# Yalt8826/WeatherForecast_STGCN_MAML

Measured on AMD Instinct MI355X. Metric: MAML meta-steps/sec (15-task batch, N=441, T=24), higher is better.
Workload: dtype f32

## Files before the change

weatherforecast_stgcn_maml_amd/_capi.py:

```python
from __future__ import annotations

import ctypes
import os
import threading

import numpy as np

HERE = os.path.dirname(os.path.abspath(__file__))
LIB_PATH = os.environ.get("SMAML_LIB") or os.path.join(HERE, "libsmaml.so")

EXPORTS = (
    "smaml_last_error", "smaml_abi_version", "smaml_build_info", "smaml_param_layout", "smaml_graph_ell",
    "smaml_create", "smaml_destroy", "smaml_set_graph", "smaml_set_gcn_params", "smaml_reserve",
    "smaml_workspace_bytes", "smaml_so_kept_steps", "smaml_set_dropout", "smaml_set_task_ids", "smaml_gcn_conv", "smaml_forward", "smaml_set_tasks",
    "smaml_meta_step", "smaml_adamw_step", "smaml_adapt_steps", "smaml_timing", "smaml_timing_collect",
    "smaml_backward", "smaml_gcn_forward", "smaml_lstm_forward", "smaml_lstm_backward", "smaml_head_loss",
    "smaml_clip_sgd", "smaml_inner_loop", "smaml_alloc", "smaml_free", "smaml_comm_unique_id",
    "smaml_comm_init", "smaml_comm_allreduce", "smaml_comm_destroy", "smaml_variant_counts", "smaml_set_option",
    "smaml_dropout", "smaml_sync", "smaml_gcn_conv_ex", "smaml_gcn_conv_backward", "smaml_relu_mask",
    "smaml_adapt_prepare", "smaml_adapt_phases",
)
ABI_VERSION = 7
GCN_RELU, GCN_PLAIN = 1, 2

VARIANTS = ("fwd", "fwd_drop", "fwd_split", "fwd_img", "fwd_dual", "fwd_dual_kept", "fwd_dual_img", "bwd_big", "bwd_small", "bwd_split",
            "bwd_dual_big", "bwd_dual_big_kept", "bwd_dual_small", "bwd_dual_small_kept", "wgrad", "wgrad_wide", "wgrad_pair",
            "fwd_kw", "bwd_kw", "gcn_dedup", "xg_dedup", "wgrad_dedup", "f_compact")

TIMING_CATEGORIES = ("gcn_layer", "lstm_fwd_step", "lstm_fwd_dual", "head_loss", "head_dh", "lstm_bwd_step",
                     "lstm_bwd_dual", "wgrad", "wgrad_reduce", "misc", "xg_proj", "dg_rowsum",
                     "lstm_fwd_step_wall", "lstm_fwd_dual_wall", "lstm_bwd_step_wall", "lstm_bwd_dual_wall")

ERRORS = {1: "EINVAL", 2: "EHIP", 3: "ENOMEM", 4: "ESTATE", 5: "ENOTIMPL"}


class SmamlError(RuntimeError):
    def __init__(self, code, msg):
        super().__init__(f"smaml error {ERRORS.get(code, code)}: {msg}")
        self.code = code


class Dims(ctypes.Structure):
    _fields_ = [(n, ctypes.c_int32) for n in (
        "num_nodes", "window_size", "input_channels", "hidden_channels", "lstm_hidden_size",
        "lstm_num_layers", "forecast_horizon", "output_channels")]

    @classmethod
    def from_model(cls, d):
        return cls(d.num_nodes, d.window_size, d.input_channels, d.hidden_channels,
                   d.lstm_hidden_size, d.lstm_num_layers, d.forecast_horizon, d.output_channels)
# ... 64 lines not shown
def lib():
    global _lib
    with _lock:
        if _lib is None:
            if not os.path.exists(LIB_PATH):
                raise SmamlError(-1, f"{LIB_PATH} not built; run __graft_entry__.build()")
            L = ctypes.CDLL(LIB_PATH)
            L.smaml_abi_version.restype = I32
            if L.smaml_abi_version() != ABI_VERSION:
                raise SmamlError(-1, f"{LIB_PATH} has ABI {L.smaml_abi_version()}, expected {ABI_VERSION}; rebuild")
            for name, (args, res) in _SIGS.items():
                fn = getattr(L, name)
                fn.argtypes = args
                fn.restype = res
            _lib = L
    return _lib


def build_info() -> str:
    return lib().smaml_build_info().decode()


def product_forms() -> dict:
    tail = build_info().split(":", 1)[1]
    return {k: int(v) for k, v in (kv.split("=") for kv in tail.split())}


def check(rc):
    if rc != 0:
        raise SmamlError(rc, lib().smaml_last_error().decode(errors="replace"))


def param_layout(dims, which: int):
    L = lib()
    d = Dims.from_model(dims)
    cap = 64
    offs = (ctypes.c_int64 * cap)()
    sizes = (ctypes.c_int64 * cap)()
    cnt = ctypes.c_int32()
    tot = ctypes.c_int64()
    check(L.smaml_param_layout(ctypes.byref(d), which, offs, sizes, cap, ctypes.byref(cnt),
                               ctypes.byref(tot)))
    return [(offs[i], sizes[i]) for i in range(cnt.value)], tot.value


def graph_ell(edge_index: np.ndarray, num_nodes: int):
    L = lib()
# ... 217 lines not shown
```

weatherforecast_stgcn_maml_amd/csrc/api.cpp:

```cpp
#include <hip/hip_runtime.h>

#include <algorithm>
#include <array>
#include <chrono>
#include <cmath>
#include <dlfcn.h>
#include <cstdlib>
#include <cstring>
#include <string>
#include <thread>
#include <vector>

#include "kernels.h"
#include "smaml.h"

using namespace smaml;

namespace {

thread_local std::string g_err;

int fail(int code, const std::string& msg) {
  g_err = msg;
  return code;
// ... 161 lines not shown
};

}

static Knobs default_knobs() {
  Knobs k;
  k.bwd_big_min = SMAML_BWD_BIG_MIN;
  k.bwdd_big_min = SMAML_BWDD_BIG_MIN;
  k.split_max = SMAML_SPLIT_MAX;
  k.wgrad_group_max_rows = SMAML_WGRAD_GROUP_ROWS;
  k.wgrad_group_wgs = SMAML_WGRAD_GROUP_WGS;
  k.gcn_fused = SMAML_GCN_FUSED;
  k.gate_img = SMAML_GATE_IMG;
  k.wgrad_wide = 1;
  k.wgrad_pair = SMAML_WGRAD_PAIR;
  k.bwdd_remap = SMAML_BWDD_REMAP_DEFAULT;
  k.small_kw = SMAML_SMALL_KW;
  k.gcn_dedup = 1;
  k.xg_dedup = SMAML_XG_DEDUP_DEFAULT;
  k.wgrad_dedup = SMAML_WGRAD_DEDUP_DEFAULT;
  k.bptt_streams = SMAML_BPTT_STREAMS_DEFAULT;
  k.fwd_streams = SMAML_FWD_STREAMS_DEFAULT;
  k.f_compact = SMAML_F_COMPACT_DEFAULT;
  return k;
}

enum { AD_RESERVE = 0, AD_ALLOC, AD_FILL, AD_STEPS, AD_NPH };
struct AdPhases {
  double ms[AD_NPH] = {};
  int64_t filled = 0;
};

struct smaml_ctx {
  smaml_dims dims{};
  Dims d{};
  ParamOff po{};
  GcnOff go{};
  int device = 0;
  int32_t* ell_c = nullptr;
  float* ell_v = nullptr;
  int32_t *tr_p = nullptr, *tr_c = nullptr;
  float* tr_v = nullptr;
  int64_t tr_nnz_cap = 0;
  float* bw_scratch = nullptr;
  int64_t bw_scratch_cap = 0;
  const float* gcn = nullptr;
// ... 1689 lines not shown
    c->kn.wgrad_group_max_rows = (int)std::min<int64_t>(value, 1 << 30);
  } else if (k == "gcn_fused" && (value == 0 || value == 1)) {
    c->kn.gcn_fused = (int)value;
  } else if (k == "gate_img" && (value == 0 || value == 1)) {
    c->kn.gate_img = (int)value;
  } else if (k == "wgrad_wide" && (value == 0 || value == 1)) {
    c->kn.wgrad_wide = (int)value;
  } else if (k == "wgrad_pair" && (value == 0 || value == 1)) {
    c->kn.wgrad_pair = (int)value;
  } else if (k == "bwdd_remap" && (value == 0 || value == 1)) {
    c->kn.bwdd_remap = (int)value;
  } else if (k == "small_kw" && value >= 0 && value <= 2) {
    c->kn.small_kw = (int)value;
  } else if (k == "gcn_dedup" && (value == 0 || value == 1)) {
    c->kn.gcn_dedup = (int)value;
  } else if (k == "xg_dedup" && (value == 0 || value == 1)) {
    c->kn.xg_dedup = (int)value;
  } else if (k == "wgrad_dedup" && (value == 0 || value == 1)) {
    c->kn.wgrad_dedup = (int)value;
  } else if (k == "bptt_streams" && value >= 1 && value <= 4) {
    c->kn.bptt_streams = (int)value;
  } else if (k == "f_compact" && (value == 0 || value == 1)) {
    c->kn.f_compact = (int)value;
  } else if (k == "fwd_streams" && value >= 0 && value <= 4) {
    c->kn.fwd_streams = (int)value;
  } else if (k == "adapt_phase_sync" && (value == 0 || value == 1)) {
    c->ad_phase_sync = (int)value;
  } else if (k == "adapt_gcn_batch" && value >= 0 && value <= 256) {
    c->ad_gcn_batch = (int)value;
  } else if (k == "wgrad_group_wgs" && value >= 1) {
    c->kn.wgrad_group_wgs = (int)std::min<int64_t>(value, 1 << 20);
  } else if (k == "grid_barrier" && (value == 0 || value == 1)) {
    c->bar_fused = (int)value;
  } else if (k == "barrier_timeout_us" && value >= 1) {
    c->bar_timeout_us = std::min<int64_t>(value, 600000000);
  } else if (k == "comm_timeout_ms" && value >= 1) {
    c->comm_timeout_ms = std::min<int64_t>(value, 3600000);
  } else if (k == "barrier_oversize" && value >= 0 && value <= 64) {
    c->bar_oversize = (int)value;
  } else if (k == "keep" && value >= -1) {
    c->keep_max = (int)std::min<int64_t>(value, 1 << 20);
    c->keep_tried_K = -1;
  } else {
    return fail(SMAML_EINVAL, "unknown option or bad value: " + k);
  }
  return SMAML_OK;
// ... 333 lines not shown
```

weatherforecast_stgcn_maml_amd/csrc/kernels.h:

```cpp
#pragma once
#include <hip/hip_runtime.h>
#include <stdint.h>

namespace smaml {

constexpr int ELLW = 8;
constexpr int MAX_LAYERS = 8;

struct Dims {
  int N = 0;
  int T = 0;
  int Cin0 = 0;
  int Hc = 0;
  int H = 0;
  int L = 0;
  int Hf = 0;
  int C = 0;
  int HfC = 0;
};

struct LayerOff {
  int64_t wih = 0, whh = 0, bih = 0, bhh = 0;
  int cin = 0;
};
// ... 39 lines not shown
  V_FWD = 0,
  V_FWD_DROP,
  V_FWD_SPLIT,
  V_FWD_IMG,
  V_FWDD,
  V_FWDD_KEPT,
  V_FWDD_IMG,
  V_BWD_BIG,
  V_BWD_SMALL,
  V_BWD_SPLIT,
  V_BWDD_BIG,
  V_BWDD_BIG_KEPT,
  V_BWDD_SMALL,
  V_BWDD_SMALL_KEPT,
  V_WGRAD,
  V_WGRAD_WIDE,
  V_WGRAD_PAIR,
  V_FWD_KW,
  V_BWD_KW,
  V_GCN_DEDUP,
  V_XG_DEDUP,
  V_WGRAD_DEDUP,
  V_F_COMPACT,
  NVAR
};

#ifndef SMAML_BWD_BIG_MIN
#define SMAML_BWD_BIG_MIN (3 * 256)
#endif
#ifndef SMAML_BWDD_BIG_MIN
#define SMAML_BWDD_BIG_MIN (3 * 256)
#endif
#ifndef SMAML_SPLIT_MAX
#define SMAML_SPLIT_MAX 4
#endif

struct Knobs {
  int bwd_big_min = 0;
  int bwdd_big_min = 0;
  int split_max = 1;
  int wgrad_group_max_rows = 0;
  int wgrad_group_wgs = 1;
  int gcn_fused = 0;
  int gate_img = 0;
  int wgrad_wide = 0;
  int wgrad_pair = 0;
  int bwdd_remap = 0;
  int small_kw = 0;
  int gcn_dedup = 0;
  int xg_dedup = 0;
  int wgrad_dedup = 0;
  int bptt_streams = 1;
  int fwd_streams = 0;
  int f_compact = 0;
};
#ifndef SMAML_GATE_IMG
#define SMAML_GATE_IMG 1
#endif
#ifndef SMAML_GCN_FUSED
#define SMAML_GCN_FUSED 1
#endif
#ifndef SMAML_BWDD_REMAP_DEFAULT
#define SMAML_BWDD_REMAP_DEFAULT 1
#endif
#ifndef SMAML_SMALL_KW
#define SMAML_SMALL_KW 1
#endif
#ifndef SMAML_XG_DEDUP_DEFAULT
#define SMAML_XG_DEDUP_DEFAULT 1
#endif
#ifndef SMAML_WGRAD_DEDUP_DEFAULT
#define SMAML_WGRAD_DEDUP_DEFAULT 1
#endif
#ifndef SMAML_BPTT_STREAMS_DEFAULT
#define SMAML_BPTT_STREAMS_DEFAULT 2
#endif
#ifndef SMAML_F_COMPACT_DEFAULT
#define SMAML_F_COMPACT_DEFAULT 1
#endif
#ifndef SMAML_FWD_STREAMS_DEFAULT
#define SMAML_FWD_STREAMS_DEFAULT 0
#endif
#ifndef SMAML_WGRAD_PAIR
#define SMAML_WGRAD_PAIR 1
#endif
#ifndef SMAML_WGRAD_GROUP_ROWS
#define SMAML_WGRAD_GROUP_ROWS 2048
#endif
#ifndef SMAML_WGRAD_GROUP_WGS
#define SMAML_WGRAD_GROUP_WGS 256
#endif

constexpr int GATE_IMG_BYTES = 3 * 128 * 16 * 2;
struct GateImgs {
  char* th = nullptr;
  char* u = nullptr;
  int64_t tstride = 0;
  int64_t off[MAX_LAYERS][2] = {};
};
constexpr int BWD_IMG_BYTES = 3 * 32 * 16 * 2;
struct BwdImgs {
// ... 97 lines not shown
inline int grid_barrier_grid(int cap, int items, int oversize) {
  if (cap <= 0 || items <= 0) return 0;
  if (oversize > 0) return cap * oversize + 1;
  const int q = cap / 4 > 0 ? cap / 4 : 1;
  return items < q ? items : q;
}
int grid_barrier_blocks(const void* fn, int items, int oversize);
int grid_barrier_capacity(const void* fn);
#ifndef SMAML_WGRAD_MAXSPLIT
#define SMAML_WGRAD_MAXSPLIT 128
#endif

struct FwdWave {
  int n = 0;
  int l[MAX_LAYERS] = {}, t[MAX_LAYERS] = {}, off[MAX_LAYERS + 1] = {};
  LayerOff lo[MAX_LAYERS] = {};
  int tm0 = 0, ntm = 0;
};
struct BwdWave {
  int n = 0;
  int l[MAX_LAYERS] = {}, t[MAX_LAYERS] = {}, off[MAX_LAYERS + 1] = {};
  LayerOff lo[MAX_LAYERS] = {};
  int64_t wih_up[MAX_LAYERS] = {};
  int tm0 = 0;
};
double bwd_wave(const Dims& d, const Work& w, const ParamOff& po, int e, int blocks_per_problem, bool dual,
                BwdWave& wv);
double fwd_wave(const Dims& d, const Work& w, const ParamOff& po, int diag, int blocks_per_problem, bool dual,
                FwdWave& wv);

const char* products_info();

void launch_gcn_layer(hipStream_t s, const Dims& d, int layer, int Zb, int B, const float* const* xtab,
                      const float* src, float* dst, bool remap_lstm, bool relu, const float* W,
                      const float* b, int cin, int cout, const int* ell_c, const float* ell_v, int rows_per_sample,
                      int ell_rows, const Drop* drop = nullptr, int drop_rps = 0);

struct FastDiv {
  uint64_t m = 0;
  uint32_t s = 0;
  uint32_t d = 0;
  FastDiv() = default;
  __host__ explicit FastDiv(uint32_t dd) : d(dd) {
    s = 0;
    while ((1ull << s) < dd) ++s;
    m = (uint64_t)((((unsigned __int128)1 << (32 + s)) + dd - 1) / dd);
  }
  __device__ __forceinline__ uint32_t div(uint32_t n) const {
    return (uint32_t)(((unsigned __int128)n * m) >> (32 + s));
  }
// ... 147 lines not shown
```

weatherforecast_stgcn_maml_amd/csrc/kernels.hip:

```cpp
#include <cmath>
#include <mutex>
#include <utility>
#include <vector>

#include "kernels.h"
#include "loaders.h"

namespace smaml {

using CfgNT = GemmCfg<128, 128, 2, 2, true, true, 32, SMAML_X6_BWD>;
using CfgGate = GemmCfg<32 * SMAML_GATE_WM, 128 * SMAML_GATE_WN, SMAML_GATE_WM, SMAML_GATE_WN, true, true, SMAML_GATE_BK, SMAML_X6_GATE,
                        SMAML_GATE_NST>;
using CfgGateP = GemmCfg<128, 128 * SMAML_GATE_WN, 4, SMAML_GATE_WN, true, true, SMAML_GATE_BK, SMAML_X6_GATE>;
using CfgNN = GemmCfg<64, 128, 2, 2, true, false, SMAML_NN_BK, SMAML_X6_BWD>;
using CfgTN = GemmCfg<SMAML_TN_BM, SMAML_TN_BN, SMAML_TN_WM, SMAML_TN_WN, false, false, SMAML_TN_BK, SMAML_X6_WGRAD,
                      SMAML_TN_NST, false>;

__device__ __forceinline__ float block_sum(float v, float* red) {
#pragma unroll
  for (int o = 32; o > 0; o >>= 1) v += __shfl_xor(v, o, 64);
  const int lane = threadIdx.x & 63, wave = threadIdx.x >> 6;
  __syncthreads();
  if (lane == 0) red[wave] = v;
  __syncthreads();
// ... 1076 lines not shown
void launch_head_dh(hipStream_t s, const Dims& d, const Work& w, const float* theta, int64_t tstride,
                    const ParamOff& po) {
  dim3 grid((w.M + CfgNN::BM - 1) / CfgNN::BM, (d.H + CfgNN::BN - 1) / CfgNN::BN, w.Z);
  k_gemm_nn<<<grid, CfgNN::NTH, 0, s>>>(w.dpred, (int64_t)w.M * d.HfC, w.M, d.HfC, theta, tstride, po.wo, d.H,
                                w.dH, (int64_t)w.M * d.H);
  if (w.drop.lstm()) launch_drop_rows(s, w, d.H, w.dH, (int64_t)w.M * d.H, w.dH);
}

using CfgNNs = GemmCfg<64, 64, 2, 2, true, false, SMAML_NN_BK, SMAML_X6_BWD>;
using CfgBwd = GemmCfg<SMAML_BWD_BM, 128, SMAML_BWD_WM, SMAML_BWD_WN, true, false, SMAML_NN_BK, SMAML_X6_BWD,
                       SMAML_BWD_NST>;

double bwd_wave(const Dims& d, const Work& w, const ParamOff& po, int e, int blocks_per_problem, bool dual,
                BwdWave& wv) {
  double fl = 0.0;
  int n = 0, off = 0;
  for (int l = d.L - 1; l >= 0; --l) {
    const int t = d.T - 1 - (e - (d.L - 1 - l));
    if (t < 0 || t >= d.T) continue;
    wv.l[n] = l;
    wv.t[n] = t;
    wv.lo[n] = po.lay[l];
    wv.wih_up[n] = l + 1 < d.L ? po.lay[l + 1].wih : 0;
    wv.off[n] = off;
    off += blocks_per_problem;
    ++n;
    const int segs = (l + 1 < d.L ? 1 : 0) + (t + 1 < d.T ? 1 : 0);
    fl += (dual ? 3.0 : 1.0) * 2.0 * w.Z * w.M * 4 * d.H * d.H * segs;
  }
  wv.n = n;
  for (int q = n; q <= MAX_LAYERS; ++q) wv.off[q] = off;
  return fl;
}

#ifndef SMAML_DIAG_BWD
#define SMAML_DIAG_BWD 0
#endif
#ifndef SMAML_EPI_DEPTH
#define SMAML_EPI_DEPTH 1
#endif
template <class C>
constexpr int epi_smem_floats() {
  constexpr int E = SMAML_BWD_HALFEPI ? C::BM * C::BN / 2 : C::BM * C::BN;
  return C::SMEM_FLOATS > E ? C::SMEM_FLOATS : E;
}

// ... 93 lines not shown
    for (int h = 0; h < 2; ++h) {
      if (h) __syncthreads();
      acc_to_lds_half<CfgNN>(acc, smem, h);
      const int mh = m0 + h * HC::BM;
      if (mh + HC::BM <= M && n0 + HC::BN <= H)
        bwd_cell_<H, HC, HEAD, false>(smem, Gz, dGz, dhz, Cz, dHz, dcz, mh, n0, t, T, M);
      else
        bwd_cell_<H, HC, HEAD, true>(smem, Gz, dGz, dhz, Cz, dHz, dcz, mh, n0, t, T, M);
    }
  } else {
    acc_to_lds<CfgNN>(acc, smem);
    if (m0 + CfgNN::BM <= M && n0 + CfgNN::BN <= H)
      bwd_cell_<H, CfgNN, HEAD, false>(smem, Gz, dGz, dhz, Cz, dHz, dcz, m0, n0, t, T, M);
    else
      bwd_cell_<H, CfgNN, HEAD, true>(smem, Gz, dGz, dhz, Cz, dHz, dcz, m0, n0, t, T, M);
  }
}

template <int H, class CfgNN, bool DROP>
__global__ SMAML_BWD_ATTR __launch_bounds__(CfgNN::NTH) void k_lstm_bwd_step(const float* GsAll, float* dGAll,
                                                      float* __restrict__ dhAll, const float* __restrict__ CsAll,
                                                      const float* __restrict__ dHhead, float* __restrict__ dcAll,
                                                      int64_t lsz, const float* __restrict__ theta, int64_t tstride,
                                                      BwdWave wv, int L, int T, int M, Drop dr) {
  __shared__ float smem[epi_smem_floats<CfgNN>()];
  constexpr int G4 = 4 * H;
  const Blk bk = xcd_block();
  int mb;
  const int p = bwd_block(wv, bk.x, mb);
  mb += wv.tm0;
  const int l = wave_sel(wv.l, p), t = wave_sel(wv.t, p);
  const LayerOff lo = wave_sel(wv.lo, p);
  const int64_t wih_up = wave_sel(wv.wih_up, p);
  const int z = bk.z;
  const int m0 = mb * CfgNN::BM, n0 = bk.y * CfgNN::BN;
  const int64_t slab = (int64_t)z * T * M;
  const float* th = theta + (int64_t)z * tstride;
  const float* Gz = GsAll + (int64_t)l * lsz * 4 + slab * G4;
  float* dGz = dGAll + (int64_t)l * lsz * 4 + slab * G4;
  float* dhz = dhAll ? dhAll + (int64_t)l * lsz + slab * H : nullptr;
  const float* Cz = CsAll + (int64_t)l * lsz + slab * H;
  float* dcz = dcAll + ((int64_t)l * gridDim.z + z) * M * H;
  Acc<CfgNN> acc;
  acc.zero();
  {
    const bool up = l + 1 < L, nx = t + 1 < T;
    const float* pa = dGAll + (int64_t)(l + 1) * lsz * 4 + (slab + (int64_t)t * M) * G4;
    const float* pn = dGz + (int64_t)(t + 1) * M * G4;
    const int ns = (up ? 1 : 0) + (nx ? 1 : 0);
    if (DROP && up) {
      const XDrop xd{drop_site(dr.seed, 2, dr.step, l), dr.thr_lstm, dr.sc_lstm,
                     ((uint64_t)dr.task_id[z] * T + t) * M * H, H};
      gemm_mainloop<CfgNN>(SegKC{{pa, nullptr, nullptr, nullptr}, {G4, 0, 0, 0}, M},
                           SegMC{{th + wih_up, nullptr}, {G4, 0}, H}, m0, n0, 0, G4, acc, smem);
      drop_acc<CfgNN>(acc, xd, m0, n0);
      if (nx)
        gemm_mainloop<CfgNN>(SegKC{{pn, nullptr, nullptr, nullptr}, {G4, 0, 0, 0}, M},
                             SegMC{{th + lo.whh, nullptr}, {G4, 0}, H}, m0, n0, 0, G4, acc, smem);
    } else {
      const SegKCt<2> la{{up ? pa : pn, pn}, {G4, G4}, M};
      const SegMCt<2> lb{{up ? th + wih_up : th + lo.whh, th + lo.whh}, {G4, G4}, H};
      if (ns && SMAML_DIAG_BWD != 2) gemm_mainloop<CfgNN>(la, lb, m0, n0, 0, ns * G4, acc, smem);
    }
  }
  if (SMAML_DIAG_BWD == 1) {
    acc_to_lds<CfgNN>(acc, smem);
    if (t < 0) dGz[threadIdx.x] = smem[threadIdx.x];
    return;
  }
  if (l == L - 1 && t == T - 1)
    bwd_cell<H, CfgNN, true>(acc, smem, Gz, dGz, dhz, Cz, dHhead + (int64_t)z * M * H, dcz, m0, n0, t, T, M);
  else
    bwd_cell<H, CfgNN, false>(acc, smem, Gz, dGz, dhz, Cz, dHhead + (int64_t)z * M * H, dcz, m0, n0, t, T, M);
}

template <int H, class CfgNN>
__global__ __launch_bounds__(CfgNN::NTH) void k_lstm_bwd_part(const float* dGAll, int64_t lsz,
                                                                            const float* __restrict__ theta,
                                                                            int64_t tstride, BwdWave wv, int L, int T,
                                                                            int M, int S, float* __restrict__ part) {
  __shared__ float smem[part_smem_floats<CfgNN, SMAML_BWD_PART_NCH>()];
  constexpr int G4 = 4 * H;
  const int p = wave_index(wv, (int)blockIdx.x);
  const int l = wave_sel(wv.l, p), t = wave_sel(wv.t, p), b0 = wave_sel(wv.off, p);
// ... 110 lines not shown
    gp[3 * H] = d * tc * go * (1.f - go);
    dcz[(int64_t)m * H + j] = dct * gf;
    if (dhz) dhz[row * H + j] = d;
  }
}
#ifndef SMAML_BWD_CELL_Q
#define SMAML_BWD_CELL_Q 1
#endif

bool bwd_wave_big(const Dims& d, const Work& w, const ParamOff& po, int e) {
  BwdWave wv{};
  const int ntm = (w.M + CfgBwd::BM - 1) / CfgBwd::BM, ntn = (d.H + CfgBwd::BN - 1) / CfgBwd::BN;
  bwd_wave(d, w, po, e, ntm, false, wv);
  return (int64_t)wv.n * ntm * ntn * w.Z * (CfgBwd::BM / 64) >= w.kn.bwd_big_min;
}

void launch_lstm_bwd_wave(hipStream_t s, const Dims& d, const Work& w, int e, const float* theta, int64_t tstride,
                          const ParamOff& po, int chunk, int nch) {
  const int64_t lsz = (int64_t)w.Z * d.T * w.M * d.H;
  BwdWave wv{};
  const int ntm = (w.M + CfgBwd::BM - 1) / CfgBwd::BM, ntn = (d.H + CfgBwd::BN - 1) / CfgBwd::BN;
  bwd_wave(d, w, po, e, ntm, false, wv);
  if (wv.n == 0) return;
#define SMAML_BWD_STEP(CFG, D_)                                                                               \
  SMAML_DISPATCH_H(d.H, k_lstm_bwd_step<HT, CFG, D_><<<grid, CFG::NTH, 0, s>>>(                                  \
                            w.Gs, w.dG, w.dh, w.Cs, w.dH, w.dc, lsz, theta, tstride, wv, d.L, d.T, w.M, w.drop))
  if (nch > 1) {
    const int lo = (int)((int64_t)ntm * chunk / nch), hi = (int)((int64_t)ntm * (chunk + 1) / nch);
    if (hi <= lo) return;
    bwd_wave(d, w, po, e, hi - lo, false, wv);
    wv.tm0 = lo;
    count_variant(w, V_BWD_BIG);
    dim3 grid(wv.off[wv.n], ntn, w.Z);
    if (w.drop.lstm()) {
      SMAML_BWD_STEP(CfgBwd, true);
    } else {
      SMAML_BWD_STEP(CfgBwd, false);
    }
    return;
  }
  const bool big = (int64_t)wv.n * ntm * ntn * w.Z * (CfgBwd::BM / 64) >= w.kn.bwd_big_min;
  if (big) {
    count_variant(w, V_BWD_BIG);
    dim3 grid(wv.off[wv.n], ntn, w.Z);
    if (w.drop.lstm()) {
      SMAML_BWD_STEP(CfgBwd, true);
    } else {
      SMAML_BWD_STEP(CfgBwd, false);
    }
  } else {
    const int ntms = (w.M + CfgNNs::BM - 1) / CfgNNs::BM, ntns = (d.H + CfgNNs::BN - 1) / CfgNNs::BN;
    bwd_wave(d, w, po, e, ntms, false, wv);
    dim3 grid(wv.off[wv.n], ntns, w.Z);
    if (!w.drop.lstm()) {
      constexpr int64_t PER = CfgNNs::WTM * CfgNNs::WTN * 16 * CfgNNs::NTH;
      const int S = small_grid_splits((int64_t)grid.x * ntns * w.Z, 8 * d.H, CfgNNs::BK,
                                      (int64_t)grid.x * ntns * w.Z * PER, w.wpart_floats, w.kn.split_max);
      if (S > 1 && small_kw_ok(d, w)) {
        launch_lstm_bwd_kw(s, d, w, e, theta, tstride, po);
        return;
      }
      if (S > 1) {
        count_variant(w, V_BWD_SPLIT);
        dim3 gp(grid.x, S * ntns, w.Z);
        SMAML_DISPATCH_H(d.H, (k_lstm_bwd_part<HT, CfgNNs><<<gp, CfgNNs::NTH, 0, s>>>(w.dG, lsz, theta, tstride, wv,
                                                                                       d.L, d.T, w.M, S, w.wpart)));
        if (SMAML_BWD_CELL_Q) {
// ... 859 lines not shown
    v[i] = vi;
  }
}

void launch_adam_l2(hipStream_t s, float* p, const float* g, float* m, float* v, int64_t n, double* part,
                    const float* lr_dev, int step, float b1, float b2, float eps, float wd, float max_norm,
                    const float* lpart, int lblocks, float inv_count, float* loss) {
  int nb = (int)((n + NT - 1) / NT);
  if (nb > 2048) nb = 2048;
  k_sqsum<<<dim3(SQB, 1), NT, 0, s>>>(g, n, part);
  const double bc1 = 1.0 - std::pow((double)b1, step), bc2 = 1.0 - std::pow((double)b2, step);
  k_adam_l2<<<nb, NT, 0, s>>>(p, g, m, v, n, part, lr_dev, bc1, (float)std::sqrt(bc2), b1, b2, eps, wd, max_norm,
                              lpart, lblocks, inv_count, loss);
}

}

namespace smaml {
template <class C>
constexpr int product_form() {
  return C::X6S ? 2 : C::X6 ? 1 : 0;
}
const char* products_info() {
  static char buf[256];
  snprintf(buf, sizeof buf,
           "products(0=f32 MFMA, 1=bf16x6 fragment split, 2=bf16x6 staged split): gcn=%d gate=%d gate_dual=%d "
           "bptt=%d bptt_dual=%d wgrad=%d",
           product_form<CfgGcn>(), product_form<CfgGate>(), SMAML_X6_GATED ? (SMAML_X6_GATED == 2 ? 2 : 1) : 0,
           product_form<CfgBwd>(), SMAML_X6_BWDD ? (SMAML_X6_BWDD == 2 ? 2 : 1) : 0, product_form<CfgTN>());
  return buf;
}
}
```

weatherforecast_stgcn_maml_amd/csrc/kernels_dual.hip:

```cpp
#include "kernels.h"
#include "loaders.h"

namespace smaml {

#ifndef SMAML_DUAL_BK
#define SMAML_DUAL_BK 16
#endif
using CfgGateD = GemmCfg<32 * SMAML_GATED_WM, 128 * SMAML_GATE_WN, SMAML_GATED_WM, SMAML_GATE_WN, true, true, SMAML_GATE_BK, SMAML_X6_GATED,
                         SMAML_GATE_NST>;
using CfgNTD = GemmCfg<128, 128, 2, 2, true, true, SMAML_DUAL_BK, SMAML_X6_BWDD>;
using CfgNND = GemmCfg<64, 128, 2, 2, true, false, SMAML_DUAL_BK, SMAML_X6_BWDD>;

__device__ __forceinline__ float block_sum_f(float v, float* red) {
#pragma unroll
  for (int o = 32; o > 0; o >>= 1) v += __shfl_xor(v, o, 64);
  const int lane = threadIdx.x & 63, wave = threadIdx.x >> 6;
  __syncthreads();
  if (lane == 0) red[wave] = v;
  __syncthreads();
  float s = 0.f;
  if (threadIdx.x == 0)
    for (int i = 0; i < NT / 64; ++i) s += red[i];
  return s;
}
// ... 526 lines not shown
      const float o1 = rdct * cp * sf + dct * rcp * sf + dct * cp * (1.f - 2.f * gf) * rf;
      const float o2 = rdct * gi * sg + dct * ri * sg - 2.f * dct * gi * gg * rgg;
      const float o3 = rdh * tc * so + dh * rtc * so + dh * tc * (1.f - 2.f * go) * ro;
      const float d0 = dct * gf, d1 = rdct * gf + dct * rf;
      if (e == 0) { o[0].x = o0; o[1].x = o1; o[2].x = o2; o[3].x = o3; odc.x = d0; ordc.x = d1; }
      if (e == 1) { o[0].y = o0; o[1].y = o1; o[2].y = o2; o[3].y = o3; odc.y = d0; ordc.y = d1; }
      if (e == 2) { o[0].z = o0; o[1].z = o1; o[2].z = o2; o[3].z = o3; odc.z = d0; ordc.z = d1; }
      if (e == 3) { o[0].w = o0; o[1].w = o1; o[2].w = o2; o[3].w = o3; odc.w = d0; ordc.w = d1; }
    }
    float* rp = RGz + (tM + m) * G4 + j;
#pragma unroll
    for (int g = 0; g < 4; ++g) st4_<SMAML_NT_BWDD != 0>(rp + g * H, o[g]);
    st4_<SMAML_NT_BWDD != 0>(dcz + (int64_t)m * H + j, odc);
    st4_<SMAML_NT_BWDD != 0>(rdcz + (int64_t)m * H + j, ordc);
  };
  V v;
#pragma unroll 1
  for (int k = 0; k < NIT; ++k) {
    load(k, v);
    step(k, v);
  }
}

struct PairRemap {
  int on;
  int Z, R, seg, NS;
};
__device__ __forceinline__ bool remap_pair(const PairRemap& rm, int Lid, int& p, int& z, int& mb) {
  const int x = Lid & 7, j = Lid >> 3;
  const int slot = j / rm.seg, rin = j - slot * rm.seg;
  const int g = x + 8 * slot;
  if (g >= rm.NS) return false;
  p = g / (2 * rm.Z);
  z = (g >> 1) % rm.Z;
  mb = (g & 1) * rm.seg + rin;
  return mb < rm.R;
}

template <int H, class CfgNND, bool KEPT, bool DROP>
__global__ SMAML_BWDD_ATTR __launch_bounds__(CfgNND::NTH) void k_lstm_bwd_dual(const float* GsAll, float* dGAll,
                                                      const float* __restrict__ dhAll, float* __restrict__ RGsAll,
                                                      const float* __restrict__ CsAll, const float* __restrict__ RCsAll,
                                                      const float* __restrict__ dHhead, const float* __restrict__ RdHhead,
                                                      float* __restrict__ dcAll, float* __restrict__ RdcAll,
                                                      int64_t lsz, const float* __restrict__ theta,
                                                      const float* __restrict__ U, int64_t tstride, BwdWave wv, int L,
                                                      int T, int M, Drop dr, PairRemap rm) {
  __shared__ float smem[bwdd_smem_floats<CfgNND>()];
  constexpr int G4 = 4 * H;
  int mb, p, z, ny;
  if (rm.on) {
    if (!remap_pair(rm, (int)blockIdx.x, p, z, mb)) return;
    ny = 0;
  } else {
    const Blk bk = xcd_block();
    p = bwd_block(wv, bk.x, mb);
    z = bk.z;
    ny = bk.y;
  }
  mb += wv.tm0;
  const int Zt = rm.on ? rm.Z : (int)gridDim.z;
  const int l = wave_sel(wv.l, p), t = wave_sel(wv.t, p);
  const LayerOff lo = wave_sel(wv.lo, p);
  const int64_t wih_up = wave_sel(wv.wih_up, p);
  const int m0 = mb * CfgNND::BM, n0 = ny * CfgNND::BN;
  const int64_t slab = (int64_t)z * T * M;
  const float* th = theta + (int64_t)z * tstride;
  const float* u = U + (int64_t)z * tstride;
  const float* Gz = GsAll + (int64_t)l * lsz * 4 + slab * G4;
  float* dGz = dGAll + (int64_t)l * lsz * 4 + slab * G4;
  float* RGz = RGsAll + (int64_t)l * lsz * 4 + slab * G4;
  const float* dhz = dhAll + (int64_t)l * lsz + slab * H;
  const float* Cz = CsAll + (int64_t)l * lsz + slab * H;
  const float* RCz = RCsAll + (int64_t)l * lsz + slab * H;
  float* dcz = dcAll + ((int64_t)l * Zt + z) * M * H;
// ... 6 lines not shown
    const int64_t oa = (int64_t)(l + 1) * lsz * 4 + (slab + (int64_t)t * M) * G4;
    const int64_t on = (int64_t)(t + 1) * M * G4;
    const int ns = (up ? 1 : 0) + (nx ? 1 : 0);
    const int w0 = ns >= 1 ? G4 : 0, w1 = ns >= 2 ? G4 : 0;
    SegKC la{{up ? dGAll + oa : dGz + on, up ? dGz + on : nullptr, nullptr, nullptr}, {w0, w1, 0, 0}, M};
    SegKC la2{{up ? RGsAll + oa : RGz + on, up ? RGz + on : nullptr, nullptr, nullptr}, {w0, w1, 0, 0}, M};
    SegMC lb{{up ? th + wih_up : th + lo.whh, th + lo.whh}, {w0, w1}, H};
    SegMC lb2{{up ? u + wih_up : u + lo.whh, u + lo.whh}, {w0, w1}, H};
    if (DROP && up) {
      const XDrop xd{drop_site(dr.seed, 2, dr.step, l), dr.thr_lstm, dr.sc_lstm,
                     ((uint64_t)dr.task_id[z] * T + t) * M * H, H};
      gemm_dual_mainloop<CfgNND, !KEPT>(SegKC{{dGAll + oa, nullptr, nullptr, nullptr}, {G4, 0, 0, 0}, M},
                                        SegKC{{RGsAll + oa, nullptr, nullptr, nullptr}, {G4, 0, 0, 0}, M},
                                        SegMC{{th + wih_up, nullptr}, {G4, 0}, H},
                                        SegMC{{u + wih_up, nullptr}, {G4, 0}, H}, m0, n0, G4, 0, ap, at, smem);
      if (!KEPT) drop_acc<CfgNND>(ap, xd, m0, n0);
      drop_acc<CfgNND>(at, xd, m0, n0);
      if (nx)
        gemm_dual_mainloop<CfgNND, !KEPT>(SegKC{{dGz + on, nullptr, nullptr, nullptr}, {G4, 0, 0, 0}, M},
                                          SegKC{{RGz + on, nullptr, nullptr, nullptr}, {G4, 0, 0, 0}, M},
                                          SegMC{{th + lo.whh, nullptr}, {G4, 0}, H},
                                          SegMC{{u + lo.whh, nullptr}, {G4, 0}, H}, m0, n0, G4, 0, ap, at, smem);
    } else if (ns && SMAML_DIAG_BWDD != 2) {
      const float* a0 = up ? dGAll + oa : dGz + on;
      const float* r0 = up ? RGsAll + oa : RGz + on;
      const int64_t w0o = up ? wih_up : lo.whh;
      gemm_dual_mainloop<CfgNND, !KEPT>(SegKCt<2, SMAML_NT_BWDD != 0>{{a0, dGz + on}, {G4, G4}, M},
                                        SegKCt<2, SMAML_NT_BWDD != 0>{{r0, RGz + on}, {G4, G4}, M},
                                        SegMCt<2>{{th + w0o, th + lo.whh}, {G4, G4}, H},
                                        SegMCt<2>{{u + w0o, u + lo.whh}, {G4, G4}, H}, m0, n0, ns * G4, 0, ap, at,
                                        smem);
    }
  }
  const bool first = (t == T - 1);
  const bool head = first && l == L - 1;
  const float* dHz = dHhead + (int64_t)z * M * H;
  const float* RdHz = RdHhead + (int64_t)z * M * H;
  const bool full = m0 + CfgNND::BM <= M;
  if constexpr (KEPT) {
    constexpr bool HALF = SMAML_BWDD_HALFEPI && CfgNND::WAVES_M == 2;
    using EC = std::conditional_t<HALF, HalfRows<CfgNND>, CfgNND>;
#pragma unroll 1
    for (int hh = 0; hh < (HALF ? 2 : 1); ++hh) {
      if (hh) __syncthreads();
      if constexpr (HALF)
        acc_to_lds_half<CfgNND>(at, smem, hh);
      else
        acc_to_lds<CfgNND>(at, smem);
      if (SMAML_DIAG_BWDD == 1) {
        if (t < 0) RGz[threadIdx.x] = smem[threadIdx.x];
        continue;
      }
      const int mh = m0 + hh * EC::BM;
// ... 41 lines not shown
      const float rdct = rdcin + rdh * go * s2 + dh * ro * s2 - 2.f * dh * go * tc * rtc;
      const float si = gi * (1.f - gi), sf = gf * (1.f - gf), so = go * (1.f - go), sg = 1.f - gg * gg;
      if (!KEPT) {
        stb(dGz, 4u * (og), dct * gg * si);
        stb(dGz, 4u * (og + H), dct * cp * sf);
        stb(dGz, 4u * (og + 2 * H), dct * gi * sg);
        stb(dGz, 4u * (og + 3 * H), dh * tc * so);
      }
      stb(RGz, 4u * (og), rdct * gg * si + dct * rgg * si + dct * gg * (1.f - 2.f * gi) * ri);
      stb(RGz, 4u * (og + H), rdct * cp * sf + dct * rcp * sf + dct * cp * (1.f - 2.f * gf) * rf);
      stb(RGz, 4u * (og + 2 * H), rdct * gi * sg + dct * ri * sg - 2.f * dct * gi * gg * rgg);
      stb(RGz, 4u * (og + 3 * H), rdh * tc * so + dh * rtc * so + dh * tc * (1.f - 2.f * go) * ro);
      stb(dcz, 4u * (oc), dct * gf);
      stb(rdcz, 4u * (oc), rdct * gf + dct * rf);
    }
  }
}

template <class Cfg, bool KEPT>
static void bwd_dual_grid(hipStream_t s, const Dims& d, const Work& w, const BwdWave& wv, int ntn, const float* theta,
                          const float* U, int64_t tstride) {
  const int64_t lsz = (int64_t)w.Z * d.T * w.M * d.H;
  dim3 grid(wv.off[wv.n], ntn, w.Z);
  PairRemap rm{};
  const int R = wv.n > 0 ? wv.off[1] - wv.off[0] : 0;
  if (w.kn.bwdd_remap && ntn == 1 && R >= 2) {
    rm.on = 1;
    rm.Z = w.Z;
    rm.R = R;
    rm.seg = (R + 1) / 2;
    rm.NS = wv.n * w.Z * 2;
    grid = dim3((unsigned)(8 * ((rm.NS + 7) / 8) * rm.seg), 1, 1);
  }
  const float* dh = KEPT ? w.dh : w.Gs;
  if (w.drop.lstm()) {
    SMAML_DISPATCH_H(d.H, k_lstm_bwd_dual<HT, Cfg, KEPT, true><<<grid, Cfg::NTH, 0, s>>>(
                              w.Gs, w.dG, dh, w.RGs, w.Cs, w.RCs, w.dH, w.RdH, w.dc, w.Rdc, lsz, theta, U, tstride,
                              wv, d.L, d.T, w.M, w.drop, rm));
  } else {
    SMAML_DISPATCH_H(d.H, k_lstm_bwd_dual<HT, Cfg, KEPT, false><<<grid, Cfg::NTH, 0, s>>>(
                              w.Gs, w.dG, dh, w.RGs, w.Cs, w.RCs, w.dH, w.RdH, w.dc, w.Rdc, lsz, theta, U, tstride,
                              wv, d.L, d.T, w.M, w.drop, rm));
  }
}

bool bwd_dual_wave_big(const Dims& d, const Work& w, const ParamOff& po, int e) {
  BwdWave wv{};
  const int ntm = (w.M + CfgBwdD::BM - 1) / CfgBwdD::BM, ntn = (d.H + CfgBwdD::BN - 1) / CfgBwdD::BN;
  bwd_wave(d, w, po, e, ntm, true, wv);
  return (int64_t)wv.n * ntm * ntn * w.Z * (CfgBwdD::BM / 64) >= w.kn.bwdd_big_min;
}

void launch_lstm_bwd_dual_wave(hipStream_t s, const Dims& d, const Work& w, int e, const float* theta,
                               const float* U, int64_t tstride, const ParamOff& po, int chunk, int nch) {
  BwdWave wv{};
// ... 117 lines not shown
```

Measured before the change: 0.6223.

## Co-locate paired BPTT wavefront problems on the same XCD and swap segment order

Generalizes the pair remap of backward LSTM blocks into a group remap that places blocks from two adjacent wavefront problems (layers sharing a weight matrix or activation slab) onto the same XCD slot. Odd layers also swap the order of their two GEMM K-segments, so co-resident blocks read shared operands at the same time. The aim is more L2 reuse of shared weights and gradients across the two problems in the serial BPTT steps. The cost is more complex block-index arithmetic, possibly more idle blocks from padding, and a new path that is skipped when LSTM dropout is on.

```diff
diff --git a/weatherforecast_stgcn_maml_amd/_capi.py b/weatherforecast_stgcn_maml_amd/_capi.py
--- a/weatherforecast_stgcn_maml_amd/_capi.py
+++ b/weatherforecast_stgcn_maml_amd/_capi.py
@@ -25,7 +25,7 @@
 
 VARIANTS = ("fwd", "fwd_drop", "fwd_split", "fwd_img", "fwd_dual", "fwd_dual_kept", "fwd_dual_img", "bwd_big", "bwd_small", "bwd_split",
             "bwd_dual_big", "bwd_dual_big_kept", "bwd_dual_small", "bwd_dual_small_kept", "wgrad", "wgrad_wide", "wgrad_pair",
-            "fwd_kw", "bwd_kw", "gcn_dedup", "xg_dedup", "wgrad_dedup", "f_compact")
+            "fwd_kw", "bwd_kw", "gcn_dedup", "xg_dedup", "wgrad_dedup", "f_compact", "bwd_coloc", "bwd_dual_coloc")
 
 TIMING_CATEGORIES = ("gcn_layer", "lstm_fwd_step", "lstm_fwd_dual", "head_loss", "head_dh", "lstm_bwd_step",
                      "lstm_bwd_dual", "wgrad", "wgrad_reduce", "misc", "xg_proj", "dg_rowsum",
@@ -136,7 +136,7 @@
 
 
 def product_forms() -> dict:
-    tail = build_info().split(":", 1)[1]
+    tail = build_info().split(":", 1)[1].split(";", 1)[0]
     return {k: int(v) for k, v in (kv.split("=") for kv in tail.split())}
 
 
diff --git a/weatherforecast_stgcn_maml_amd/csrc/api.cpp b/weatherforecast_stgcn_maml_amd/csrc/api.cpp
--- a/weatherforecast_stgcn_maml_amd/csrc/api.cpp
+++ b/weatherforecast_stgcn_maml_amd/csrc/api.cpp
@@ -207,6 +207,8 @@
   k.bptt_streams = SMAML_BPTT_STREAMS_DEFAULT;
   k.fwd_streams = SMAML_FWD_STREAMS_DEFAULT;
   k.f_compact = SMAML_F_COMPACT_DEFAULT;
+  k.bptt_seg_order = SMAML_BPTT_SEG_ORDER_DEFAULT;
+  k.bptt_coloc = SMAML_BPTT_COLOC_DEFAULT;
   return k;
 }
 
@@ -1942,6 +1944,10 @@
     c->kn.bptt_streams = (int)value;
   } else if (k == "f_compact" && (value == 0 || value == 1)) {
     c->kn.f_compact = (int)value;
+  } else if (k == "bptt_seg_order" && (value == 0 || value == 1)) {
+    c->kn.bptt_seg_order = (int)value;
+  } else if (k == "bptt_coloc" && value >= 0 && value <= 3) {
+    c->kn.bptt_coloc = (int)value;
   } else if (k == "fwd_streams" && value >= 0 && value <= 4) {
     c->kn.fwd_streams = (int)value;
   } else if (k == "adapt_phase_sync" && (value == 0 || value == 1)) {
diff --git a/weatherforecast_stgcn_maml_amd/csrc/kernels.h b/weatherforecast_stgcn_maml_amd/csrc/kernels.h
--- a/weatherforecast_stgcn_maml_amd/csrc/kernels.h
+++ b/weatherforecast_stgcn_maml_amd/csrc/kernels.h
@@ -85,6 +85,8 @@
   V_XG_DEDUP,
   V_WGRAD_DEDUP,
   V_F_COMPACT,
+  V_BWD_COLOC,
+  V_BWDD_COLOC,
   NVAR
 };
 
@@ -116,6 +118,8 @@
   int bptt_streams = 1;
   int fwd_streams = 0;
   int f_compact = 0;
+  int bptt_seg_order = 0;
+  int bptt_coloc = 0;
 };
 #ifndef SMAML_GATE_IMG
 #define SMAML_GATE_IMG 1
@@ -140,6 +144,12 @@
 #endif
 #ifndef SMAML_F_COMPACT_DEFAULT
 #define SMAML_F_COMPACT_DEFAULT 1
+#endif
+#ifndef SMAML_BPTT_SEG_ORDER_DEFAULT
+#define SMAML_BPTT_SEG_ORDER_DEFAULT 1
+#endif
+#ifndef SMAML_BPTT_COLOC_DEFAULT
+#define SMAML_BPTT_COLOC_DEFAULT 3
 #endif
 #ifndef SMAML_FWD_STREAMS_DEFAULT
 #define SMAML_FWD_STREAMS_DEFAULT 0
@@ -283,10 +293,54 @@
   int l[MAX_LAYERS] = {}, t[MAX_LAYERS] = {}, off[MAX_LAYERS + 1] = {};
   LayerOff lo[MAX_LAYERS] = {};
   int64_t wih_up[MAX_LAYERS] = {};
+  int nxf[MAX_LAYERS] = {};
   int tm0 = 0;
 };
 double bwd_wave(const Dims& d, const Work& w, const ParamOff& po, int e, int blocks_per_problem, bool dual,
                 BwdWave& wv);
+
+struct GroupRemap {
+  int on = 0;
+  int n = 0, Z = 0, R = 0;
+  int grp = 1, seg = 0, nseg = 0;
+  int NS = 0;
+};
+inline GroupRemap group_remap(int n, int Z, int R, int grp) {
+  GroupRemap rm{};
+  if (n <= 0 || Z <= 0 || R < 1 || grp < 1 || (grp == 1 && R < 2)) return rm;
+  rm.on = 1;
+  rm.n = n;
+  rm.Z = Z;
+  rm.R = R;
+  rm.grp = grp;
+  const int cap = 96 / grp, units = (n + grp - 1) / grp * Z;
+  rm.nseg = grp == 1 ? 2 : (R + cap - 1) / cap;
+  if (grp > 1)
+    for (int q = rm.nseg; q <= 8 * rm.nseg && 4 * q <= R; ++q)
+      if (units * q % 8 == 0) {
+        rm.nseg = q;
+        break;
+      }
+  rm.seg = (R + rm.nseg - 1) / rm.nseg;
+  rm.nseg = (R + rm.seg - 1) / rm.seg;
+  rm.NS = units * rm.nseg;
+  return rm;
+}
+inline int64_t group_remap_grid(const GroupRemap& rm) { return (int64_t)8 * ((rm.NS + 7) / 8) * rm.seg * rm.grp; }
+__host__ __device__ inline bool remap_group(const GroupRemap& rm, int Lid, int& p, int& z, int& mb) {
+  const int x = Lid & 7, j = Lid >> 3;
+  const int per = rm.seg * rm.grp;
+  const int slot = j / per, jin = j - slot * per;
+  const int g = x + 8 * slot;
+  if (g >= rm.NS) return false;
+  const int rin = jin / rm.grp, which = jin - rin * rm.grp;
+  const int gz = g / rm.nseg, s = g - gz * rm.nseg;
+  const int pg = gz / rm.Z;
+  z = gz - pg * rm.Z;
+  p = pg * rm.grp + which;
+  mb = s * rm.seg + rin;
+  return p < rm.n && mb < rm.R;
+}
 double fwd_wave(const Dims& d, const Work& w, const ParamOff& po, int diag, int blocks_per_problem, bool dual,
                 FwdWave& wv);
 
diff --git a/weatherforecast_stgcn_maml_amd/csrc/kernels.hip b/weatherforecast_stgcn_maml_amd/csrc/kernels.hip
--- a/weatherforecast_stgcn_maml_amd/csrc/kernels.hip
+++ b/weatherforecast_stgcn_maml_amd/csrc/kernels.hip
@@ -1122,6 +1122,7 @@
     wv.t[n] = t;
     wv.lo[n] = po.lay[l];
     wv.wih_up[n] = l + 1 < d.L ? po.lay[l + 1].wih : 0;
+    wv.nxf[n] = (w.kn.bptt_seg_order && (l & 1)) ? 1 : 0;
     wv.off[n] = off;
     off += blocks_per_problem;
     ++n;
@@ -1261,25 +1262,32 @@
                                                       float* __restrict__ dhAll, const float* __restrict__ CsAll,
                                                       const float* __restrict__ dHhead, float* __restrict__ dcAll,
                                                       int64_t lsz, const float* __restrict__ theta, int64_t tstride,
-                                                      BwdWave wv, int L, int T, int M, Drop dr) {
+                                                      BwdWave wv, int L, int T, int M, Drop dr, GroupRemap rm) {
   __shared__ float smem[epi_smem_floats<CfgNN>()];
   constexpr int G4 = 4 * H;
-  const Blk bk = xcd_block();
-  int mb;
-  const int p = bwd_block(wv, bk.x, mb);
+  int mb, p, z, ny;
+  if (rm.on) {
+    if (!remap_group(rm, (int)blockIdx.x, p, z, mb)) return;
+    ny = 0;
+  } else {
+    const Blk bk = xcd_block();
+    p = bwd_block(wv, bk.x, mb);
+    z = bk.z;
+    ny = bk.y;
+  }
   mb += wv.tm0;
+  const int Zt = rm.on ? rm.Z : (int)gridDim.z;
   const int l = wave_sel(wv.l, p), t = wave_sel(wv.t, p);
   const LayerOff lo = wave_sel(wv.lo, p);
   const int64_t wih_up = wave_sel(wv.wih_up, p);
-  const int z = bk.z;
-  const int m0 = mb * CfgNN::BM, n0 = bk.y * CfgNN::BN;
+  const int m0 = mb * CfgNN::BM, n0 = ny * CfgNN::BN;
   const int64_t slab = (int64_t)z * T * M;
   const float* th = theta + (int64_t)z * tstride;
   const float* Gz = GsAll + (int64_t)l * lsz * 4 + slab * G4;
   float* dGz = dGAll + (int64_t)l * lsz * 4 + slab * G4;
   float* dhz = dhAll ? dhAll + (int64_t)l * lsz + slab * H : nullptr;
   const float* Cz = CsAll + (int64_t)l * lsz + slab * H;
-  float* dcz = dcAll + ((int64_t)l * gridDim.z + z) * M * H;
+  float* dcz = dcAll + ((int64_t)l * Zt + z) * M * H;
   Acc<CfgNN> acc;
   acc.zero();
   {
@@ -1297,8 +1305,10 @@
         gemm_mainloop<CfgNN>(SegKC{{pn, nullptr, nullptr, nullptr}, {G4, 0, 0, 0}, M},
                              SegMC{{th + lo.whh, nullptr}, {G4, 0}, H}, m0, n0, 0, G4, acc, smem);
     } else {
-      const SegKCt<2> la{{up ? pa : pn, pn}, {G4, G4}, M};
-      const SegMCt<2> lb{{up ? th + wih_up : th + lo.whh, th + lo.whh}, {G4, G4}, H};
+      const bool sw = up && nx && wave_sel(wv.nxf, p) != 0;
+      const bool ab0 = up && !sw;
+      const SegKCt<2> la{{ab0 ? pa : pn, sw ? pa : pn}, {G4, G4}, M};
+      const SegMCt<2> lb{{ab0 ? th + wih_up : th + lo.whh, sw ? th + wih_up : th + lo.whh}, {G4, G4}, H};
       if (ns && SMAML_DIAG_BWD != 2) gemm_mainloop<CfgNN>(la, lb, m0, n0, 0, ns * G4, acc, smem);
     }
   }
@@ -1455,9 +1465,17 @@
   const int ntm = (w.M + CfgBwd::BM - 1) / CfgBwd::BM, ntn = (d.H + CfgBwd::BN - 1) / CfgBwd::BN;
   bwd_wave(d, w, po, e, ntm, false, wv);
   if (wv.n == 0) return;
+  GroupRemap rm{};
+  auto coloc_grid = [&](dim3& grid) {
+    if (!((w.kn.bptt_coloc & 1) && w.kn.bptt_seg_order) || w.drop.lstm() || ntn != 1 || wv.n < 2) return;
+    rm = group_remap(wv.n, w.Z, wv.off[1] - wv.off[0], 2);
+    if (!rm.on) return;
+    grid = dim3((unsigned)group_remap_grid(rm), 1, 1);
+    count_variant(w, V_BWD_COLOC);
+  };
 #define SMAML_BWD_STEP(CFG, D_)                                                                               \
   SMAML_DISPATCH_H(d.H, k_lstm_bwd_step<HT, CFG, D_><<<grid, CFG::NTH, 0, s>>>(                                  \
-                            w.Gs, w.dG, w.dh, w.Cs, w.dH, w.dc, lsz, theta, tstride, wv, d.L, d.T, w.M, w.drop))
+                            w.Gs, w.dG, w.dh, w.Cs, w.dH, w.dc, lsz, theta, tstride, wv, d.L, d.T, w.M, w.drop, rm))
   if (nch > 1) {
     const int lo = (int)((int64_t)ntm * chunk / nch), hi = (int)((int64_t)ntm * (chunk + 1) / nch);
     if (hi <= lo) return;
@@ -1465,6 +1483,7 @@
     wv.tm0 = lo;
     count_variant(w, V_BWD_BIG);
     dim3 grid(wv.off[wv.n], ntn, w.Z);
+    coloc_grid(grid);
     if (w.drop.lstm()) {
       SMAML_BWD_STEP(CfgBwd, true);
     } else {
@@ -1476,6 +1495,7 @@
   if (big) {
     count_variant(w, V_BWD_BIG);
     dim3 grid(wv.off[wv.n], ntn, w.Z);
+    coloc_grid(grid);
     if (w.drop.lstm()) {
       SMAML_BWD_STEP(CfgBwd, true);
     } else {
@@ -2381,12 +2401,13 @@
   return C::X6S ? 2 : C::X6 ? 1 : 0;
 }
 const char* products_info() {
-  static char buf[256];
+  static char buf[320];
   snprintf(buf, sizeof buf,
            "products(0=f32 MFMA, 1=bf16x6 fragment split, 2=bf16x6 staged split): gcn=%d gate=%d gate_dual=%d "
-           "bptt=%d bptt_dual=%d wgrad=%d",
+           "bptt=%d bptt_dual=%d wgrad=%d; defaults: bptt_seg_order=%d bptt_coloc=%d",
            product_form<CfgGcn>(), product_form<CfgGate>(), SMAML_X6_GATED ? (SMAML_X6_GATED == 2 ? 2 : 1) : 0,
-           product_form<CfgBwd>(), SMAML_X6_BWDD ? (SMAML_X6_BWDD == 2 ? 2 : 1) : 0, product_form<CfgTN>());
+           product_form<CfgBwd>(), SMAML_X6_BWDD ? (SMAML_X6_BWDD == 2 ? 2 : 1) : 0, product_form<CfgTN>(),
+           SMAML_BPTT_SEG_ORDER_DEFAULT, SMAML_BPTT_COLOC_DEFAULT);
   return buf;
 }
 }
diff --git a/weatherforecast_stgcn_maml_amd/csrc/kernels_dual.hip b/weatherforecast_stgcn_maml_amd/csrc/kernels_dual.hip
--- a/weatherforecast_stgcn_maml_amd/csrc/kernels_dual.hip
+++ b/weatherforecast_stgcn_maml_amd/csrc/kernels_dual.hip
@@ -572,20 +572,6 @@
   }
 }
 
-struct PairRemap {
-  int on;
-  int Z, R, seg, NS;
-};
-__device__ __forceinline__ bool remap_pair(const PairRemap& rm, int Lid, int& p, int& z, int& mb) {
-  const int x = Lid & 7, j = Lid >> 3;
-  const int slot = j / rm.seg, rin = j - slot * rm.seg;
-  const int g = x + 8 * slot;
-  if (g >= rm.NS) return false;
-  p = g / (2 * rm.Z);
-  z = (g >> 1) % rm.Z;
-  mb = (g & 1) * rm.seg + rin;
-  return mb < rm.R;
-}
 
 template <int H, class CfgNND, bool KEPT, bool DROP>
 __global__ SMAML_BWDD_ATTR __launch_bounds__(CfgNND::NTH) void k_lstm_bwd_dual(const float* GsAll, float* dGAll,
@@ -595,12 +581,12 @@
                                                       float* __restrict__ dcAll, float* __restrict__ RdcAll,
                                                       int64_t lsz, const float* __restrict__ theta,
                                                       const float* __restrict__ U, int64_t tstride, BwdWave wv, int L,
-                                                      int T, int M, Drop dr, PairRemap rm) {
+                                                      int T, int M, Drop dr, GroupRemap rm) {
   __shared__ float smem[bwdd_smem_floats<CfgNND>()];
   constexpr int G4 = 4 * H;
   int mb, p, z, ny;
   if (rm.on) {
-    if (!remap_pair(rm, (int)blockIdx.x, p, z, mb)) return;
+    if (!remap_group(rm, (int)blockIdx.x, p, z, mb)) return;
     ny = 0;
   } else {
     const Blk bk = xcd_block();
@@ -653,13 +639,17 @@
                                           SegMC{{th + lo.whh, nullptr}, {G4, 0}, H},
                                           SegMC{{u + lo.whh, nullptr}, {G4, 0}, H}, m0, n0, G4, 0, ap, at, smem);
     } else if (ns && SMAML_DIAG_BWDD != 2) {
-      const float* a0 = up ? dGAll + oa : dGz + on;
-      const float* r0 = up ? RGsAll + oa : RGz + on;
-      const int64_t w0o = up ? wih_up : lo.whh;
-      gemm_dual_mainloop<CfgNND, !KEPT>(SegKCt<2, SMAML_NT_BWDD != 0>{{a0, dGz + on}, {G4, G4}, M},
-                                        SegKCt<2, SMAML_NT_BWDD != 0>{{r0, RGz + on}, {G4, G4}, M},
-                                        SegMCt<2>{{th + w0o, th + lo.whh}, {G4, G4}, H},
-                                        SegMCt<2>{{u + w0o, u + lo.whh}, {G4, G4}, H}, m0, n0, ns * G4, 0, ap, at,
+      const bool sw = up && nx && wave_sel(wv.nxf, p) != 0;
+      const bool ab0 = up && !sw;
+      const float* a0 = ab0 ? dGAll + oa : dGz + on;
+      const float* r0 = ab0 ? RGsAll + oa : RGz + on;
+      const float* a1 = sw ? dGAll + oa : dGz + on;
+      const float* r1 = sw ? RGsAll + oa : RGz + on;
+      const int64_t w0o = ab0 ? wih_up : lo.whh, w1o = sw ? wih_up : lo.whh;
+      gemm_dual_mainloop<CfgNND, !KEPT>(SegKCt<2, SMAML_NT_BWDD != 0>{{a0, a1}, {G4, G4}, M},
+                                        SegKCt<2, SMAML_NT_BWDD != 0>{{r0, r1}, {G4, G4}, M},
+                                        SegMCt<2>{{th + w0o, th + w1o}, {G4, G4}, H},
+                                        SegMCt<2>{{u + w0o, u + w1o}, {G4, G4}, H}, m0, n0, ns * G4, 0, ap, at,
                                         smem);
     }
   }
@@ -747,15 +737,13 @@
                           const float* U, int64_t tstride) {
   const int64_t lsz = (int64_t)w.Z * d.T * w.M * d.H;
   dim3 grid(wv.off[wv.n], ntn, w.Z);
-  PairRemap rm{};
+  GroupRemap rm{};
   const int R = wv.n > 0 ? wv.off[1] - wv.off[0] : 0;
-  if (w.kn.bwdd_remap && ntn == 1 && R >= 2) {
-    rm.on = 1;
-    rm.Z = w.Z;
-    rm.R = R;
-    rm.seg = (R + 1) / 2;
-    rm.NS = wv.n * w.Z * 2;
-    grid = dim3((unsigned)(8 * ((rm.NS + 7) / 8) * rm.seg), 1, 1);
+  if (w.kn.bwdd_remap && ntn == 1 && R >= 1) {
+    const bool coloc = (w.kn.bptt_coloc & 2) && w.kn.bptt_seg_order && !w.drop.lstm() && wv.n >= 2;
+    rm = group_remap(wv.n, w.Z, R, coloc ? 2 : 1);
+    if (rm.on) grid = dim3((unsigned)group_remap_grid(rm), 1, 1);
+    if (rm.on && rm.grp == 2) count_variant(w, V_BWDD_COLOC);
   }
   const float* dh = KEPT ? w.dh : w.Gs;
   if (w.drop.lstm()) {
```

Result: no change. 0.6218 (-0.1%).
